# bschrag620/PyRad

Measured on NVIDIA B200. Metric: line-gridpoint evals/s, higher is better.
Workload: dtype f32

## Files before the change

pyrad_b200/csrc/common.cuh:

```cuda
#pragma once
#include <cuda_runtime.h>
#include <stdint.h>
#include <math.h>

namespace prb {

constexpr double kBoltz = 1.38064852E-23;
constexpr double cLight = 299792458.0;
constexpr double hPlanck = 6.62607004e-34;
constexpr double kPi = 3.141592653589793;
constexpr double kT0 = 296.0;
constexpr double kP0 = 1013.25;
constexpr double kAvogadro = 6.022140857E23;

constexpr int REGIME_GAUSS = 0, REGIME_LORENTZ = 1, REGIME_VOIGT = 2;

struct GroupParams {
    double conc;
    double dopp;
    double qratio;
    double weight;
};

struct DevState {
    unsigned int reserved0;
    unsigned int flags;
    unsigned int tile_counter;
    unsigned int pad;
};

constexpr unsigned int FLAG_OVERFLOW = 1u, FLAG_NONFINITE = 2u;

#ifndef PRB_K2_CONSUMERS
#define PRB_K2_CONSUMERS 8
#endif
#ifndef PRB_K2_ACC_SMEM
#define PRB_K2_ACC_SMEM 0
#endif
constexpr int K2_CONSUMERS = PRB_K2_CONSUMERS;
constexpr int K2_THREADS = 32 * (K2_CONSUMERS + 1);
#ifndef PRB_K2_CHUNK
#define PRB_K2_CHUNK 768
#endif
#ifndef PRB_K2_STAGES
#define PRB_K2_STAGES 3
#endif
#ifndef PRB_K2_MIN_CTAS
#define PRB_K2_MIN_CTAS 2
#endif
constexpr int K2_CHUNK = PRB_K2_CHUNK;
constexpr int K2_STAGES = PRB_K2_STAGES;
constexpr int K2_MIN_CTAS = PRB_K2_MIN_CTAS;
constexpr int K2_FLUSH = 64;
constexpr float K2_SENTINEL = 3.0e38f;

__device__ __forceinline__ uint32_t smem_u32(const void *p) {
    return (uint32_t)__cvta_generic_to_shared(p);
}
__device__ __forceinline__ void mbar_init(uint64_t *bar, uint32_t count) {
    asm volatile("mbarrier.init.shared::cta.b64 [%0], %1;" ::"r"(smem_u32(bar)), "r"(count) : "memory");
}
__device__ __forceinline__ void mbar_expect_tx(uint64_t *bar, uint32_t bytes) {
    asm volatile("mbarrier.arrive.expect_tx.shared::cta.b64 _, [%0], %1;" ::"r"(smem_u32(bar)), "r"(bytes)
                 : "memory");
}
__device__ __forceinline__ void mbar_arrive(uint64_t *bar) {
    asm volatile("mbarrier.arrive.shared::cta.b64 _, [%0];" ::"r"(smem_u32(bar)) : "memory");
}
__device__ __forceinline__ void mbar_wait(uint64_t *bar, uint32_t parity) {
    asm volatile(
        "{\n"
        ".reg .pred p;\n"
        "WAIT_%=:\n"
        "mbarrier.try_wait.parity.shared::cta.b64 p, [%0], %1;\n"
        "@p bra DONE_%=;\n"
        "bra WAIT_%=;\n"
        "DONE_%=:\n"
        "}\n" ::"r"(smem_u32(bar)),
        "r"(parity)
        : "memory");
}
__device__ __forceinline__ void mbar_wait_parked(uint64_t *bar, uint32_t parity) {
    asm volatile(
        "{\n"
        ".reg .pred p;\n"
        "WAITP_%=:\n"
        "mbarrier.try_wait.parity.shared::cta.b64 p, [%0], %1, %2;\n"
        "@p bra DONEP_%=;\n"
        "bra WAITP_%=;\n"
        "DONEP_%=:\n"
        "}\n" ::"r"(smem_u32(bar)),
        "r"(parity), "r"(4000u)
        : "memory");
}
__device__ __forceinline__ void tma_bulk_g2s(void *dst, const void *src, uint32_t bytes, uint64_t *bar) {
    asm volatile(
        "cp.async.bulk.shared::cluster.global.mbarrier::complete_tx::bytes [%0], [%1], %2, [%3];" ::"r"(
            smem_u32(dst)),
        "l"(src), "r"(bytes), "r"(smem_u32(bar))
        : "memory");
}

}
```

pyrad_b200/csrc/k2_line_sum.cuh:

```cuda
#pragma once
#include "common.cuh"
#include "k3_stream.cuh"

namespace prb {

__device__ __forceinline__ float rcp_approx(float x) {
    float r;
    asm("rcp.approx.ftz.f32 %0, %1;" : "=f"(r) : "f"(x));
    return r;
}
__device__ __forceinline__ float ex2_approx(float x) {
    float r;
    asm("ex2.approx.ftz.f32 %0, %1;" : "=f"(r) : "f"(x));
    return r;
}

__device__ __forceinline__ void tma_bulk_s2g(void *dst, const void *src, uint32_t bytes) {
    asm volatile("cp.async.bulk.global.shared::cta.bulk_group [%0], [%1], %2;" ::"l"(dst), "r"(smem_u32(src)), "r"(bytes)
                 : "memory");
}
__device__ __forceinline__ void consumer_barrier() {
    asm volatile("bar.sync 1, %0;" ::"n"(K2_CONSUMERS * 32) : "memory");
}

__device__ __forceinline__ int warp_lower_bound(const int32_t *__restrict__ idx, int lo, int hi, long long key) {
    const int lane = threadIdx.x & 31;
    while (hi > lo) {
        const int span = hi - lo;
        const int step = (span + 31) >> 5;
        int pos = lo + (lane + 1) * step - 1;
        pos = pos < hi - 1 ? pos : hi - 1;
        const bool less = (long long)__ldg(idx + pos) < key;
        const unsigned m = __ballot_sync(0xffffffffu, less);
        const int c = __popc(m);
        int nlo = lo, nhi = hi;
        if (c > 0) { int p = lo + c * step - 1; p = p < hi - 1 ? p : hi - 1; nlo = p + 1; }
        if (c < 32) { int p = lo + (c + 1) * step - 1; p = p < hi - 1 ? p : hi - 1; nhi = p; }
        lo = nlo;
        hi = nhi;
    }
    return lo;
}

constexpr int K2_MAX_XSC = 8;
struct K2Layer {
    const float4 *recA;
    const float4 *recB;
    const float *recD;
    void *out;
    double inv_scale;
    int l_begin, l_end;
    int wm;
    int pad;
    double xsc_w[K2_MAX_XSC];
};

constexpr int K2_MAX_PEERS = 8;
constexpr int K2_MAX_DST = K2_MAX_PEERS + 1;
struct K2Fuse {
    int enabled;
    int n_dst;
    float neg_depth_log2e;
    float c2_over_t, c2_over_tsurf;
    long long n_total;
    double x0, dx, x_last;
    float *rad[K2_MAX_DST];
    float *trans[K2_MAX_DST];
};

struct K2Args {
    const K2Layer *layers;
    int n_layers;
    const int32_t *idx;
    long long i_begin;
    int n_chunk;
    int n_tiles;
    int tile_base;
    const int2 *tile_bounds;
    int variant;
    int out_mode;
    DevState *st;
    K2Fuse fuse;
    const double *far_lag;
    float far_delta[16];
    const double *far_lag2;
    float far_delta2[16];
    const double *xsc_sigma;
    long long xsc_ld;
    int n_xsc;
    int parts;
    double *part_sums;
    unsigned int *part_count;
};

__device__ __forceinline__ double k2_add_xsc(const K2Args &a, const K2Layer *L, int i, double v) {
    for (int t = 0; t < a.n_xsc; ++t)
        v = __dadd_rn(v, __dmul_rn(__ldg(a.xsc_sigma + (long long)t * a.xsc_ld + i), __ldg(&L->xsc_w[t])));
    return v;
}

constexpr int K2_FAR_NODES = 16;
constexpr int K2_FAR_RADIUS_SPANS = 1;
constexpr int K2_FAR_SUBGROUPS = 64 / K2_FAR_NODES;
constexpr int K2_FAR_FLUSH = 16;
#ifndef PRB_K2_FAR2_SPANS
#define PRB_K2_FAR2_SPANS 8
#endif
constexpr int K2_FAR2_SPANS = PRB_K2_FAR2_SPANS;
#ifndef PRB_K2_FAR2_ENABLE
#define PRB_K2_FAR2_ENABLE 1
#endif
constexpr bool K2_FAR2 = PRB_K2_FAR2_ENABLE != 0;
constexpr int K2_FAR2_MIN_DOMAINS = 4;
static_assert(K2_CONSUMERS % K2_FAR2_SPANS == 0, "a tile is a whole number of level-2 domains");

struct K2Desc {
    int tile0;
    int cnt;
    int flags;
    int layer;
    int part;
};
constexpr int K2_FIRST = 1, K2_LAST = 2, K2_END = 4;

struct K2Smem {
    float4 rA[K2_STAGES][K2_CHUNK];
    float4 rB[K2_STAGES][K2_CHUNK];
    float rD[K2_STAGES][K2_CHUNK];
    K2Desc desc[K2_STAGES];
    uint64_t full[K2_STAGES];
    uint64_t empty[K2_STAGES];
    double far2[2][K2_CONSUMERS][K2_FAR_NODES];
    double2 faracc[2][K2_CONSUMERS * 32];
    int part_last;
};

template <int P>
__host__ __device__ constexpr size_t K2_SMEM_BASE() {
    return ((sizeof(K2Smem) + (PRB_K2_ACC_SMEM ? sizeof(double) * P * K2_CONSUMERS * 32 : 0)) + 127) & ~size_t(127);
}
template <int P>
__host__ __device__ constexpr size_t K2_SMEM_BYTES(bool peer_staging) {
    return K2_SMEM_BASE<P>() + (peer_staging ? sizeof(float) * 2 * K2_CONSUMERS * 32 * P : 0);
}

template <int H>
struct Acc {
    float2 fi[H];
    float2 a32[H];
#if PRB_K2_ACC_SMEM
    double *a64;
    __device__ __forceinline__ double &acc(int p) { return a64[p * (K2_CONSUMERS * 32)]; }
#else
    double a64[2 * H];
    __device__ __forceinline__ double &acc(int p) { return a64[p]; }
#endif
    __device__ __forceinline__ void flush() {
#pragma unroll
        for (int j = 0; j < H; ++j) {
            acc(2 * j) += (double)a32[j].x;
            acc(2 * j + 1) += (double)a32[j].y;
            a32[j] = make_float2(0.f, 0.f);
        }
    }
};

__device__ __forceinline__ float2 splat(float v) { return make_float2(v, v); }
__device__ __forceinline__ float2 lo2(const float4 &v) { return make_float2(v.x, v.y); }
__device__ __forceinline__ float2 hi2(const float4 &v) { return make_float2(v.z, v.w); }

template <int H, bool MASKED>
__device__ __forceinline__ void triple_step(const float4 &a1, const float4 &a2, const float4 &a3, const float2 &B1,
                                            const float2 &B2, const float2 &B3, float wmf, Acc<H> &s) {
    const float2 nf1 = lo2(a1), nf2 = lo2(a2), nf3 = lo2(a3);
#pragma unroll
    for (int h = 0; h < H; ++h) {
        const float2 e1 = __fadd2_rn(s.fi[h], nf1);
        const float2 e2 = __fadd2_rn(s.fi[h], nf2);
        const float2 e3 = __fadd2_rn(s.fi[h], nf3);
        const float2 q1 = __ffma2_rn(e1, e1, B1);
        const float2 q2 = __ffma2_rn(e2, e2, B2);
        const float2 q3 = __ffma2_rn(e3, e3, B3);
        float2 A1 = hi2(a1), A2 = hi2(a2), A3 = hi2(a3);
        if (MASKED) {
            A1.x = fabsf(e1.x) <= wmf ? A1.x : 0.f;
            A1.y = fabsf(e1.y) <= wmf ? A1.y : 0.f;
            A2.x = fabsf(e2.x) <= wmf ? A2.x : 0.f;
            A2.y = fabsf(e2.y) <= wmf ? A2.y : 0.f;
            A3.x = fabsf(e3.x) <= wmf ? A3.x : 0.f;
            A3.y = fabsf(e3.y) <= wmf ? A3.y : 0.f;
        }
        const float2 p23 = __fmul2_rn(q2, q3);
        const float2 t = __ffma2_rn(A3, q2, __fmul2_rn(A2, q3));
        const float2 num = __ffma2_rn(q1, t, __fmul2_rn(A1, p23));
        const float2 den = __fmul2_rn(q1, p23);
        const float2 r = make_float2(rcp_approx(den.x), rcp_approx(den.y));
        s.a32[h] = __ffma2_rn(num, r, s.a32[h]);
    }
}

__device__ __forceinline__ float2 ldB(const float4 *sB, int j) { return *reinterpret_cast<const float2 *>(sB + j); }

template <int H, bool MASKED>
__device__ __forceinline__ void lorentz_paired(const float4 *sA, const float4 *sB, int js, int je, float wmf,
                                               Acc<H> &s) {
    const int n = je - js;
    if (n <= 0) return;
    int j = js;
    const int n6 = (n / 6) * 6;
    const int jq = js + n6;
    if (n6) {
        float4 xa1 = sA[j], xa2 = sA[j + 1], xa3 = sA[j + 2], ya1 = sA[j + 3], ya2 = sA[j + 4], ya3 = sA[j + 5];
        float2 xb1 = ldB(sB, j), xb2 = ldB(sB, j + 1), xb3 = ldB(sB, j + 2);
        float2 yb1 = ldB(sB, j + 3), yb2 = ldB(sB, j + 4), yb3 = ldB(sB, j + 5);
        int since = 0;
        for (j += 6; j < jq; j += 6) {
            triple_step<H, MASKED>(xa1, xa2, xa3, xb1, xb2, xb3, wmf, s);
            xa1 = sA[j]; xa2 = sA[j + 1]; xa3 = sA[j + 2];
            xb1 = ldB(sB, j); xb2 = ldB(sB, j + 1); xb3 = ldB(sB, j + 2);
            triple_step<H, MASKED>(ya1, ya2, ya3, yb1, yb2, yb3, wmf, s);
            ya1 = sA[j + 3]; ya2 = sA[j + 4]; ya3 = sA[j + 5];
            yb1 = ldB(sB, j + 3); yb2 = ldB(sB, j + 4); yb3 = ldB(sB, j + 5);
            if (++since == K2_FLUSH / 6) { s.flush(); since = 0; }
        }
        triple_step<H, MASKED>(xa1, xa2, xa3, xb1, xb2, xb3, wmf, s);
        triple_step<H, MASKED>(ya1, ya2, ya3, yb1, yb2, yb3, wmf, s);
    }
    for (j = jq; j < je; j += 3) {
        const float4 a1 = sA[j];
        const float2 B1 = ldB(sB, j);
        const float4 z = make_float4(a1.x, a1.y, 0.f, 0.f);
        const bool h2 = j + 1 < je, h3 = j + 2 < je;
        triple_step<H, MASKED>(a1, h2 ? sA[j + 1] : z, h3 ? sA[j + 2] : z, B1, h2 ? ldB(sB, j + 1) : B1,
                               h3 ? ldB(sB, j + 2) : B1, wmf, s);
    }
    s.flush();
}

#ifndef PRB_K2_GAUSS_PAIR_H
#define PRB_K2_GAUSS_PAIR_H 2
#endif
constexpr int K2_GAUSS_PAIR_H = PRB_K2_GAUSS_PAIR_H;

template <int H, bool MASKED>
__device__ __forceinline__ void gauss_pass(const float4 *sA, const float4 *sB, const float *sD, int js, int je,
                                           float wbf, float we1f, float wmf, Acc<H> &s) {
    int since = 0;
    for (int jb = js; jb < je; jb += 32) {
        const int jt = jb + (int)(threadIdx.x & 31);
        bool hit = false;
        if (jt < je) {
            const float dg = sD[jt];
            const float f = -sA[jt].x;
            hit = (dg >= 0.f) && (f + dg >= wbf) && (f - dg <= we1f);
        }
        unsigned int m = __ballot_sync(0xffffffffu, hit);
        auto one = [&](const float4 &b, float nf1) {
            const float2 nf = splat(nf1), C2 = splat(b.w);
#pragma unroll
            for (int h = 0; h < H; ++h) {
                const float2 e = __fadd2_rn(s.fi[h], nf);
                const float2 arg = __fmul2_rn(C2, __fmul2_rn(e, e));
                float2 g = splat(b.z);
                if (MASKED) {
                    g.x = fabsf(e.x) <= wmf ? b.z : 0.f;
                    g.y = fabsf(e.y) <= wmf ? b.z : 0.f;
                }
                s.a32[h] = __ffma2_rn(g, make_float2(ex2_approx(arg.x), ex2_approx(arg.y)), s.a32[h]);
            }
        };
        while (m) {
            const int j = jb + __ffs(m) - 1;
            m &= m - 1;
            if (H <= K2_GAUSS_PAIR_H && m) {
                const int j2 = jb + __ffs(m) - 1;
                m &= m - 1;
                const float4 b1 = sB[j], b2 = sB[j2];
                const float n1 = sA[j].x, n2 = sA[j2].x;
                const float2 nfa = splat(n1), nfb = splat(n2), Ca = splat(b1.w), Cb = splat(b2.w);
                float2 ta[H], tb[H], ga[H], gb[H];
#pragma unroll
                for (int h = 0; h < H; ++h) {
                    const float2 ea = __fadd2_rn(s.fi[h], nfa), eb = __fadd2_rn(s.fi[h], nfb);
                    const float2 xa = __fmul2_rn(Ca, __fmul2_rn(ea, ea)), xb = __fmul2_rn(Cb, __fmul2_rn(eb, eb));
                    ga[h] = splat(b1.z);
                    gb[h] = splat(b2.z);
                    if (MASKED) {
                        ga[h].x = fabsf(ea.x) <= wmf ? b1.z : 0.f;
                        ga[h].y = fabsf(ea.y) <= wmf ? b1.z : 0.f;
                        gb[h].x = fabsf(eb.x) <= wmf ? b2.z : 0.f;
                        gb[h].y = fabsf(eb.y) <= wmf ? b2.z : 0.f;
                    }
                    ta[h] = make_float2(ex2_approx(xa.x), ex2_approx(xa.y));
                    tb[h] = make_float2(ex2_approx(xb.x), ex2_approx(xb.y));
                }
#pragma unroll
                for (int h = 0; h < H; ++h) s.a32[h] = __ffma2_rn(gb[h], tb[h], __ffma2_rn(ga[h], ta[h], s.a32[h]));
                since += 2;
                if (since >= K2_FLUSH) { s.flush(); since = 0; }
                continue;
            }
            one(sB[j], sA[j].x);
            if (++since >= K2_FLUSH) { s.flush(); since = 0; }
        }
    }
    if (since) s.flush();
}

struct FarAcc {
    double v0, v1;
};
__device__ __forceinline__ float2 far_triple(const float4 &a1, const float4 &a2, const float4 &a3, const float2 &B1,
                                             const float2 &B2, const float2 &B3, const float2 &A1, const float2 &A2,
                                             const float2 &A3, const float2 &wb2, const float2 &del, const float2 &part) {
    const float2 e1 = __fadd2_rn(__fadd2_rn(wb2, lo2(a1)), del);
    const float2 e2 = __fadd2_rn(__fadd2_rn(wb2, lo2(a2)), del);
    const float2 e3 = __fadd2_rn(__fadd2_rn(wb2, lo2(a3)), del);
    const float2 q1 = __ffma2_rn(e1, e1, B1);
    const float2 q2 = __ffma2_rn(e2, e2, B2);
    const float2 q3 = __ffma2_rn(e3, e3, B3);
    const float2 p23 = __fmul2_rn(q2, q3);
    const float2 t = __ffma2_rn(A3, q2, __fmul2_rn(A2, q3));
    const float2 num = __ffma2_rn(q1, t, __fmul2_rn(A1, p23));
    const float2 den = __fmul2_rn(q1, p23);
    const float2 r = make_float2(rcp_approx(den.x), rcp_approx(den.y));
    return __ffma2_rn(num, r, part);
}
template <int G>
__device__ __forceinline__ void far_pass(const float4 *sA, const float4 *sB, int js, int je, float wbf, float2 del,
                                         double2 *acc, int sub) {
    const int n = je - js;
    if (n <= 0) return;
    const double2 acc0 = *acc;
    FarAcc fa{acc0.x, acc0.y};
    const float2 wb2 = splat(wbf);
    const float2 zero = make_float2(0.f, 0.f);
    int full = n / (3 * G);
    const float4 *pa = sA + js + sub;
    const float4 *pb = sB + js + sub;
    while (full > 0) {
        const int m = min(full, K2_FAR_FLUSH);
        float2 part = zero;
#pragma unroll 2
        for (int i = 0; i < m; ++i) {
            const float4 a1 = pa[0], a2 = pa[G], a3 = pa[2 * G];
            const float2 B1 = ldB(pb, 0), B2 = ldB(pb, G), B3 = ldB(pb, 2 * G);
            part = far_triple(a1, a2, a3, B1, B2, B3, hi2(a1), hi2(a2), hi2(a3), wb2, del, part);
            pa += 3 * G;
            pb += 3 * G;
        }
        fa.v0 += (double)part.x;
        fa.v1 += (double)part.y;
        full -= m;
    }
    const int j0 = js + (n / (3 * G)) * (3 * G);
    if (j0 < je) {
        const int j1 = j0 + sub, j2 = j1 + G, j3 = j1 + 2 * G;
        const int k1 = min(j1, je - 1), k2 = min(j2, je - 1), k3 = min(j3, je - 1);
        const float4 a1 = sA[k1], a2 = sA[k2], a3 = sA[k3];
        const float2 A1 = j1 < je ? hi2(a1) : zero, A2 = j2 < je ? hi2(a2) : zero, A3 = j3 < je ? hi2(a3) : zero;
        const float2 part = far_triple(a1, a2, a3, ldB(sB, k1), ldB(sB, k2), ldB(sB, k3), A1, A2, A3, wb2, del, zero);
        fa.v0 += (double)part.x;
        fa.v1 += (double)part.y;
    }
    *acc = make_double2(fa.v0, fa.v1);
}

template <int H>
__device__ __forceinline__ void general_all(const float4 *sA, const float4 *sB, int cnt, float wmf, Acc<H> &s) {
    for (int jb = 0; jb < cnt; jb += K2_FLUSH) {
        const int jend = min(jb + K2_FLUSH, cnt);
        for (int j = jb; j < jend; ++j) {
            const float4 a = sA[j], b = sB[j];
#pragma unroll
            for (int h = 0; h < H; ++h) {
                const float ex = s.fi[h].x + a.x, ey = s.fi[h].y + a.x;
                const float e2x = ex * ex, e2y = ey * ey;
                float tx = a.z * rcp_approx(e2x + b.x), ty = a.z * rcp_approx(e2y + b.x);
                tx = fmaf(b.z, ex2_approx(b.w * e2x), tx);
                ty = fmaf(b.z, ex2_approx(b.w * e2y), ty);
                s.a32[h].x += (fabsf(ex) <= wmf) ? tx : 0.f;
                s.a32[h].y += (fabsf(ey) <= wmf) ? ty : 0.f;
            }
        }
        s.flush();
    }
}

template <int P, bool FAR, bool SPLIT>
__device__ __forceinline__ void k2_line_sum_body(const K2Args &a) {
    static_assert(P >= 2 && P % 2 == 0, "points per thread must be even (packed FP32x2)");
    static_assert(!FAR || P == 4 || P == 8, "far-field tables exist for 128- and 256-point spans");
    constexpr int H = P / 2;
    constexpr int TILE = K2_CONSUMERS * 32 * P;
    constexpr int SPAN = 32 * P;
    extern __shared__ __align__(128) unsigned char smem_raw[];
    K2Smem &sm = *reinterpret_cast<K2Smem *>(smem_raw);
    const int tid = threadIdx.x, lane = tid & 31, warp = tid >> 5;

    if (tid == 0) {
        for (int s = 0; s < K2_STAGES; ++s) {
            mbar_init(&sm.full[s], 1);
            mbar_init(&sm.empty[s], K2_CONSUMERS);
        }
        asm volatile("fence.mbarrier_init.release.cluster;" ::: "memory");
        asm volatile("fence.proxy.async.shared::cta;" ::: "memory");
    }
    __syncthreads();

    if (warp == K2_CONSUMERS) {
        uint32_t it = 0;
        auto slot_acquire = [&](uint32_t &stage) {
            stage = it % K2_STAGES;
            mbar_wait_parked(&sm.empty[stage], ((it / K2_STAGES) & 1) ^ 1);
        };
        const int parts = (SPLIT && a.parts > 1) ? a.parts : 1;
        const int n_items = a.n_layers * a.n_tiles * parts;
        while (true) {
            int item = 0;
            if (lane == 0) item = (int)atomicAdd(&a.st->tile_counter, 1u);
            item = __shfl_sync(0xffffffffu, item, 0);
            if (item >= n_items) break;
            const int n_lt = a.n_layers * a.n_tiles;
            const int pidx = item / n_lt;
            const int lt = item - pidx * n_lt;
            const int half = parts >> 1, step = pidx >> 2, r = pidx & 3;
            const int part = parts < 4 ? pidx : (r == 0 ? half - 1 - step : r == 1 ? half + step : r == 2 ? step : parts - 1 - step);
            const int layer = lt / a.n_tiles;
            const int tile = a.tile_base + lt - layer * a.n_tiles;
            const K2Layer *L = a.layers + layer;
            const int wm = __ldg(&L->wm), l_begin = __ldg(&L->l_begin), l_end = __ldg(&L->l_end);
            const float4 *recA = L->recA;
            const float4 *recB = L->recB;
            const float *recD = L->recD;
            const int tile0 = tile * TILE;
            const long long k_lo = a.i_begin + tile0 - wm;
            const long long k_hi = a.i_begin + tile0 + TILE - 1 + wm + 1;
            int lo = warp_lower_bound(a.idx, l_begin, l_end, k_lo);
            const int hi = warp_lower_bound(a.idx, lo, l_end, k_hi);
            lo &= ~3;
            const int nch = hi > lo ? (hi - lo + K2_CHUNK - 1) / K2_CHUNK : 1;
            const int c0 = (int)((long long)part * nch / parts), c1 = (int)((long long)(part + 1) * nch / parts);
            const int cn = c1 > c0 ? c1 - c0 : 1;
            for (int k = 0; k < cn; ++k, ++it) {
                const int c = c0 + k;
                uint32_t stage;
                slot_acquire(stage);
                if (lane == 0) {
                    const int first = lo + c * K2_CHUNK;
                    const int cnt = c1 > c0 ? max(min(K2_CHUNK, hi - first), 0) : 0;
                    sm.desc[stage] = K2Desc{tile0, cnt, (k == 0 ? K2_FIRST : 0) | (k == cn - 1 ? K2_LAST : 0), layer, part};
                    if (cnt > 0) {
                        const uint32_t ce = (uint32_t)((cnt + 3) & ~3);
                        mbar_expect_tx(&sm.full[stage], ce * 36u);
                        tma_bulk_g2s(sm.rA[stage], recA + first, ce * 16u, &sm.full[stage]);
                        tma_bulk_g2s(sm.rB[stage], recB + first, ce * 16u, &sm.full[stage]);
                        tma_bulk_g2s(sm.rD[stage], recD + first, ce * 4u, &sm.full[stage]);
                    } else {
                        mbar_arrive(&sm.full[stage]);
                    }
                }
                __syncwarp();
            }
        }
        uint32_t stage;
        slot_acquire(stage);
        if (lane == 0) {
            sm.desc[stage] = K2Desc{0, 0, K2_END, 0, 0};
            mbar_arrive(&sm.full[stage]);
        }
        return;
    }

    float wmf = 0.f;
    Acc<H> s;
#pragma unroll
    for (int h = 0; h < H; ++h) { s.a32[h] = make_float2(0.f, 0.f); s.fi[h] = make_float2(0.f, 0.f); }
#if PRB_K2_ACC_SMEM
    s.a64 = reinterpret_cast<double *>(smem_raw + sizeof(K2Smem)) + tid;
#endif
#pragma unroll
    for (int p = 0; p < P; ++p) s.acc(p) = 0.0;
    int wb = 0;
    float wbf = 0.f, we1f = 0.f;
    double2 *far = &sm.faracc[0][tid];
    double2 *far2 = &sm.faracc[1][tid];
    float dbf = 0.f;
    uint32_t tile_par = 0;
    bool use2 = false;

    for (uint32_t it = 0;; ++it) {
        const uint32_t stage = it % K2_STAGES;
        mbar_wait(&sm.full[stage], (it / K2_STAGES) & 1);
        const K2Desc d = sm.desc[stage];
        if (d.flags & K2_END) {
            if (tid == 0) asm volatile("cp.async.bulk.wait_group 0;" ::: "memory");
            break;
        }
        if (d.flags & K2_FIRST) {
            wmf = (float)__ldg(&a.layers[d.layer].wm);
            wb = d.tile0 + warp * SPAN;
            wbf = (float)wb;
            we1f = (float)(wb + SPAN - 1);
#pragma unroll
            for (int h = 0; h < H; ++h) {
                s.a32[h] = make_float2(0.f, 0.f);
                s.fi[h] = make_float2((float)(wb + lane + 64 * h), (float)(wb + lane + 64 * h + 32));
            }
#pragma unroll
            for (int p = 0; p < P; ++p) s.acc(p) = 0.0;
            if (FAR) {
                *far = make_double2(0.0, 0.0);
                *far2 = make_double2(0.0, 0.0);
            }
            dbf = (float)(d.tile0 + (warp / K2_FAR2_SPANS) * (K2_FAR2_SPANS * SPAN));
            use2 = FAR && K2_FAR2 && wmf >= (float)(K2_FAR2_MIN_DOMAINS * K2_FAR2_SPANS * SPAN);
        }
        const int cnt = d.cnt;
        const float4 *sA = sm.rA[stage];
        const float4 *sB = sm.rB[stage];
        const float *sD = sm.rD[stage];

        if (a.variant == 0) {
            general_all<H>(sA, sB, cnt, wmf, s);
        } else if (cnt > 0) {
            float dgl = 0.f;
            for (int j = lane; j < cnt; j += 32) dgl = fmaxf(dgl, sD[j]);
            const float dgmax = __uint_as_float(__reduce_max_sync(0xffffffffu, __float_as_uint(dgl)));
            const float t0 = wbf - wmf;
            const float t5 = we1f + 1.f + wmf;
            float t1 = we1f - wmf, t4 = wbf + wmf + 1.f;
            if (t1 >= t4) { t1 = t5; t4 = t5; }
            const float g0 = fmaxf(wbf - dgmax, t0);
            const float g1 = fminf(we1f + 1.f + dgmax, t5);
            const float tfl = wbf + (float)((SPAN - 1) / 2 - K2_FAR_RADIUS_SPANS * SPAN);
            const float tfr = wbf + (float)(SPAN / 2 + K2_FAR_RADIUS_SPANS * SPAN);
            int b1, b4, bg0, bg1;
            if (FAR) {
                static_assert(K2_CHUNK <= 1024, "one level-1 sample per lane");
                const float f1 = -sA[min(32 * lane + 31, cnt - 1)].x;
                const bool v1 = 32 * lane < cnt;
                auto below = [&](float t) -> int {
                    const int nb = __popc(__ballot_sync(0xffffffffu, v1 && f1 < t));
                    const int j2 = 32 * nb + lane;
                    const bool l2 = j2 < cnt && -sA[min(j2, cnt - 1)].x < t;
                    return min(32 * nb, cnt) + __popc(__ballot_sync(0xffffffffu, l2));
                };
                constexpr int S2 = K2_FAR2_SPANS * SPAN;
                const int kp = lane & (K2_FAR_NODES / 2 - 1);
                const int sub = lane / (K2_FAR_NODES / 2);
                const float2 del = make_float2(a.far_delta[2 * kp], a.far_delta[2 * kp + 1]);
                const float2 del2 = make_float2(a.far_delta2[2 * kp], a.far_delta2[2 * kp + 1]);
                const int sub2 = (warp % K2_FAR2_SPANS) * K2_FAR_SUBGROUPS + sub;
                const float u1 = dbf + (float)(S2 - 1) - wmf, u4 = dbf + wmf + 1.f;
                const bool l2on = use2 && u1 < u4;
                b1 = below(t1);
                lorentz_paired<H, true>(sA, sB, below(t0), b1, wmf, s);
                b4 = below(t4);
                const int bfl = min(max(below(tfl), b1), b4);
                if (l2on) {
                    const int c4 = below(u4);
                    const int c1 = min(below(u1), c4);
                    const int cfl = min(max(below(dbf + (float)((S2 - 1) / 2 - K2_FAR_RADIUS_SPANS * S2)), c1), c4);
                    const int l1a = min(max(c1, b1), bfl), l1b = min(max(cfl, l1a), bfl);
                    far_pass<K2_FAR_SUBGROUPS>(sA, sB, b1, l1a, wbf, del, far, sub);
                    far_pass<K2_FAR2_SPANS * K2_FAR_SUBGROUPS>(sA, sB, c1, cfl, dbf, del2, far2, sub2);
                    far_pass<K2_FAR_SUBGROUPS>(sA, sB, l1b, bfl, wbf, del, far, sub);
                } else {
                    far_pass<K2_FAR_SUBGROUPS>(sA, sB, b1, bfl, wbf, del, far, sub);
                }
                const int bfr = min(max(below(tfr + 1.f), bfl), b4);
                lorentz_paired<H, false>(sA, sB, bfl, bfr, wmf, s);
                if (l2on) {
                    const int c4 = below(u4);
                    const int c1 = min(below(u1), c4);
                    const int cfl = min(max(below(dbf + (float)((S2 - 1) / 2 - K2_FAR_RADIUS_SPANS * S2)), c1), c4);
                    const int cfr = min(max(below(dbf + (float)(S2 / 2 + K2_FAR_RADIUS_SPANS * S2) + 1.f), cfl), c4);
                    const int r1a = min(max(cfr, bfr), b4), r1b = min(max(c4, r1a), b4);
                    far_pass<K2_FAR_SUBGROUPS>(sA, sB, bfr, r1a, wbf, del, far, sub);
                    far_pass<K2_FAR2_SPANS * K2_FAR_SUBGROUPS>(sA, sB, cfr, c4, dbf, del2, far2, sub2);
                    far_pass<K2_FAR_SUBGROUPS>(sA, sB, r1b, b4, wbf, del, far, sub);
                } else {
                    far_pass<K2_FAR_SUBGROUPS>(sA, sB, bfr, b4, wbf, del, far, sub);
                }
                lorentz_paired<H, true>(sA, sB, b4, below(t5), wmf, s);
                bg0 = below(g0);
                bg1 = below(g1);
            } else {
                int c0 = 0, c1 = 0, c4 = 0, c5 = 0, cg0 = 0, cg1 = 0;
                for (int j = lane; j < cnt; j += 32) {
                    const float f = -sA[j].x;
                    c0 += f < t0; c1 += f < t1; c4 += f < t4; c5 += f < t5; cg0 += f < g0; cg1 += f < g1;
                }
                const int b0 = __reduce_add_sync(0xffffffffu, c0);
                b1 = __reduce_add_sync(0xffffffffu, c1);
                b4 = __reduce_add_sync(0xffffffffu, c4);
                const int b5 = __reduce_add_sync(0xffffffffu, c5);
                bg0 = __reduce_add_sync(0xffffffffu, cg0);
                bg1 = __reduce_add_sync(0xffffffffu, cg1);
                lorentz_paired<H, true>(sA, sB, b0, b1, wmf, s);
                lorentz_paired<H, false>(sA, sB, b1, b4, wmf, s);
                lorentz_paired<H, true>(sA, sB, b4, b5, wmf, s);
            }
            if (dgmax > 0.f) {
                gauss_pass<H, true>(sA, sB, sD, bg0, min(bg1, b1), wbf, we1f, wmf, s);
                gauss_pass<H, false>(sA, sB, sD, max(bg0, b1), min(bg1, b4), wbf, we1f, wmf, s);
                gauss_pass<H, true>(sA, sB, sD, max(bg0, b4), bg1, wbf, we1f, wmf, s);
            }
        }
        __syncwarp();
        if (lane == 0) mbar_arrive(&sm.empty[stage]);

        if (d.flags & K2_LAST) {
            const K2Layer *L = a.layers + d.layer;
            const double inv_scale = __ldg(&L->inv_scale);
            void *out = L->out;
            const bool bulk = a.fuse.enabled && a.fuse.n_dst > 1 && d.tile0 + TILE <= a.n_chunk;
            float *stage_rad = reinterpret_cast<float *>(smem_raw + K2_SMEM_BASE<P>());
            float *stage_tr = stage_rad + TILE;
            if (bulk) {
                if (tid == 0) asm volatile("cp.async.bulk.wait_group.read 0;" ::: "memory");
                consumer_barrier();
            }
            if (FAR) {
                double v0 = far->x, v1 = far->y, w0 = far2->x, w1 = far2->y;
#pragma unroll
                for (int o = K2_FAR_NODES / 2; o < 32; o <<= 1) {
                    v0 += __shfl_xor_sync(0xffffffffu, v0, o);
                    v1 += __shfl_xor_sync(0xffffffffu, v1, o);
                    w0 += __shfl_xor_sync(0xffffffffu, w0, o);
                    w1 += __shfl_xor_sync(0xffffffffu, w1, o);
                }
                if (use2 && lane < K2_FAR_NODES / 2) {
                    sm.far2[tile_par][warp][2 * lane] = w0;
                    sm.far2[tile_par][warp][2 * lane + 1] = w1;
                }
                if (use2) consumer_barrier();
                double dn = 0.0;
                if (use2 && lane < K2_FAR_NODES) {
                    const int wd = (warp / K2_FAR2_SPANS) * K2_FAR2_SPANS;
#pragma unroll
                    for (int q = 0; q < K2_FAR2_SPANS; ++q) dn += sm.far2[tile_par][wd + q][lane];
                }
                if (use2) tile_par ^= 1u;
                constexpr int S2 = K2_FAR2_SPANS * SPAN;
                const double *lw2base = a.far_lag2 + (warp % K2_FAR2_SPANS) * SPAN + lane;
#pragma unroll 2
                for (int k = 0; k < K2_FAR_NODES; ++k) {
                    const double fk = __shfl_sync(0xffffffffu, (k & 1) ? v1 : v0, k >> 1);
                    const double *lw = a.far_lag + k * SPAN + lane;
#pragma unroll
                    for (int p = 0; p < P; ++p) s.acc(p) = fma(fk, __ldg(lw + 32 * p), s.acc(p));
                    if (use2) {
                        const double gk = __shfl_sync(0xffffffffu, dn, k);
                        const double *lw2 = lw2base + k * S2;
#pragma unroll
                        for (int p = 0; p < P; ++p) s.acc(p) = fma(gk, __ldg(lw2 + 32 * p), s.acc(p));
                    }
                }
            }
            bool finish = true;
            if (SPLIT && a.parts > 1) {
                const int lt = d.layer * a.n_tiles + (d.tile0 / TILE - a.tile_base);
                double *mine = a.part_sums + ((size_t)lt * a.parts + d.part) * TILE + warp * SPAN + lane;
#pragma unroll
                for (int p = 0; p < P; ++p) __stcg(mine + 32 * p, s.acc(p));
                __threadfence();
                consumer_barrier();
                if (tid == 0) sm.part_last = atomicAdd(a.part_count + lt, 1u) == (unsigned int)(a.parts - 1);
                consumer_barrier();
                finish = sm.part_last != 0;
                if (finish) {
                    __threadfence();
                    const double *all = a.part_sums + (size_t)lt * a.parts * TILE + warp * SPAN + lane;
#pragma unroll
                    for (int p = 0; p < P; ++p) {
                        double v = 0.0;
                        for (int q = 0; q < a.parts; ++q) v += __ldcg(all + (size_t)q * TILE + 32 * p);
                        s.acc(p) = v;
                    }
                }
            }
            if (finish) {
#pragma unroll
                for (int p = 0; p < P; ++p) {
                    const int i = wb + 32 * p + lane;
                    if (i < a.n_chunk) {
                        const double v = k2_add_xsc(a, L, i, s.acc(p) * inv_scale);
                        if (a.out_mode == 0) reinterpret_cast<double *>(out)[i] = v;
                        else reinterpret_cast<float *>(out)[i] = (float)v;
                        if (a.fuse.enabled) {
                            const double x = axis_value(a.i_begin + i, a.fuse.n_total, a.fuse.x0, a.fuse.dx, a.fuse.x_last);
                            const float nu = (float)x;
                            const float a3 = (float)(2E8 * hPlanck * (cLight * cLight) * (x * x * x));
                            const float e = (float)v * a.fuse.neg_depth_log2e;
                            const float b = planck_f32(a3, a.fuse.c2_over_t * nu);
                            const float rad = k3_fold_step(planck_f32(a3, a.fuse.c2_over_tsurf * nu), e, b);
                            const float tr = exp2f(0.f + e);
                            if (bulk) {
                                stage_rad[i - d.tile0] = rad;
                                stage_tr[i - d.tile0] = tr;
                            } else {
#pragma unroll 1
                                for (int dst = 0; dst < a.fuse.n_dst; ++dst) {
                                    a.fuse.rad[dst][i] = rad;
                                    a.fuse.trans[dst][i] = tr;
                                }
                            }
                        }
                    }
                }
                if (bulk) {
                    asm volatile("fence.proxy.async.shared::cta;" ::: "memory");
                    consumer_barrier();
                    if (tid == 0) {
#pragma unroll 1
                        for (int dst = 0; dst < a.fuse.n_dst; ++dst) {
                            tma_bulk_s2g(a.fuse.rad[dst] + d.tile0, stage_rad, TILE * 4u);
                            tma_bulk_s2g(a.fuse.trans[dst] + d.tile0, stage_tr, TILE * 4u);
                        }
                        asm volatile("cp.async.bulk.commit_group;" ::: "memory");
                    }
                }
            }
        }
    }
}

template <int P, bool SPLIT = false>
__global__ void __launch_bounds__(K2_THREADS, K2_MIN_CTAS) k2_line_sum(const K2Args a) {
    k2_line_sum_body<P, false, SPLIT>(a);
}
template <int P, bool SPLIT = false>
__global__ void __launch_bounds__(K2_THREADS, K2_MIN_CTAS) k2_line_sum_far(const K2Args a) {
    k2_line_sum_body<P, true, SPLIT>(a);
}

}
```

Measured before the change: 4990 billion.

## Offload per-slot line bounds and Gaussian hit masks to producer warp

For non-FAR paths with P>=8, the producer warp builds a per-stage index after each chunk lands. It holds binary-searched line bounds for every consumer span plus a bitmask of Gaussian hits, and publishes it through a new 'ready' mbarrier. Consumers read these precomputed bounds and masks instead of scanning all lines with per-warp counting reductions and ballots. This moves redundant per-warp work onto the otherwise idle producer warp, at the cost of extra shared memory, a serial producer stage that could delay consumers, and more complex barrier interleaving.

Measured after the change: 5053 billion, median of 6. 1.01x the previous value.

```diff
diff --git a/pyrad_b200/csrc/common.cuh b/pyrad_b200/csrc/common.cuh
--- a/pyrad_b200/csrc/common.cuh
+++ b/pyrad_b200/csrc/common.cuh
@@ -93,6 +93,19 @@
         "r"(parity), "r"(4000u)
         : "memory");
 }
+__device__ __forceinline__ bool mbar_test(uint64_t *bar, uint32_t parity) {
+    uint32_t done;
+    asm volatile(
+        "{\n"
+        ".reg .pred p;\n"
+        "mbarrier.test_wait.parity.shared::cta.b64 p, [%1], %2;\n"
+        "selp.u32 %0, 1, 0, p;\n"
+        "}\n"
+        : "=r"(done)
+        : "r"(smem_u32(bar)), "r"(parity)
+        : "memory");
+    return done != 0;
+}
 __device__ __forceinline__ void tma_bulk_g2s(void *dst, const void *src, uint32_t bytes, uint64_t *bar) {
     asm volatile(
         "cp.async.bulk.shared::cluster.global.mbarrier::complete_tx::bytes [%0], [%1], %2, [%3];" ::"r"(
diff --git a/pyrad_b200/csrc/k2_line_sum.cuh b/pyrad_b200/csrc/k2_line_sum.cuh
--- a/pyrad_b200/csrc/k2_line_sum.cuh
+++ b/pyrad_b200/csrc/k2_line_sum.cuh
@@ -123,6 +123,12 @@
 };
 constexpr int K2_FIRST = 1, K2_LAST = 2, K2_END = 4;
 
+struct K2SlotIndex {
+    int b0, b1, b4, b5, bg0, bg1;
+};
+static_assert(K2_CHUNK % 32 == 0, "Gaussian hit masks: whole 32-line words per slot");
+constexpr int K2_GMASK_WORDS = K2_CHUNK / 32;
+
 struct K2Smem {
     float4 rA[K2_STAGES][K2_CHUNK];
     float4 rB[K2_STAGES][K2_CHUNK];
@@ -130,6 +136,9 @@
     K2Desc desc[K2_STAGES];
     uint64_t full[K2_STAGES];
     uint64_t empty[K2_STAGES];
+    uint64_t ready[K2_STAGES];
+    K2SlotIndex index[K2_STAGES][K2_CONSUMERS];
+    uint32_t gmask[K2_STAGES][K2_CONSUMERS][K2_GMASK_WORDS];
     double far2[2][K2_CONSUMERS][K2_FAR_NODES];
     double2 faracc[2][K2_CONSUMERS * 32];
     int part_last;
@@ -242,19 +251,26 @@
 #endif
 constexpr int K2_GAUSS_PAIR_H = PRB_K2_GAUSS_PAIR_H;
 
-template <int H, bool MASKED>
-__device__ __forceinline__ void gauss_pass(const float4 *sA, const float4 *sB, const float *sD, int js, int je,
-                                           float wbf, float we1f, float wmf, Acc<H> &s) {
+__device__ __forceinline__ bool gauss_hit(float f, float dg, float wbf, float we1f) {
+    return (dg >= 0.f) && (f + dg >= wbf) && (f - dg <= we1f);
+}
+
+template <int H, bool MASKED, bool INDEXED>
+__device__ __forceinline__ void gauss_pass(const float4 *sA, const float4 *sB, const float *sD, const uint32_t *gm,
+                                           int js, int je, float wbf, float we1f, float wmf, Acc<H> &s) {
     int since = 0;
     for (int jb = js; jb < je; jb += 32) {
-        const int jt = jb + (int)(threadIdx.x & 31);
-        bool hit = false;
-        if (jt < je) {
-            const float dg = sD[jt];
-            const float f = -sA[jt].x;
-            hit = (dg >= 0.f) && (f + dg >= wbf) && (f - dg <= we1f);
-        }
-        unsigned int m = __ballot_sync(0xffffffffu, hit);
+        unsigned int m;
+        if (INDEXED) {
+            const int k = jb >> 5;
+            m = __funnelshift_r(gm[k], gm[min(k + 1, K2_GMASK_WORDS - 1)], jb & 31);
+            if (je - jb < 32) m &= (1u << (je - jb)) - 1u;
+        } else {
+            const int jt = jb + (int)(threadIdx.x & 31);
+            bool hit = false;
+            if (jt < je) hit = gauss_hit(-sA[jt].x, sD[jt], wbf, we1f);
+            m = __ballot_sync(0xffffffffu, hit);
+        }
         auto one = [&](const float4 &b, float nf1) {
             const float2 nf = splat(nf1), C2 = splat(b.w);
 #pragma unroll
@@ -387,6 +403,71 @@
     }
 }
 
+__device__ __forceinline__ float slot_dgmax(const float *sD, int cnt) {
+    float dgl = 0.f;
+    for (int j = (int)(threadIdx.x & 31); j < cnt; j += 32) dgl = fmaxf(dgl, sD[j]);
+    return __uint_as_float(__reduce_max_sync(0xffffffffu, __float_as_uint(dgl)));
+}
+
+struct K2Thresholds {
+    float t0, t1, t4, t5, g0, g1;
+};
+__device__ __forceinline__ K2Thresholds span_thresholds(float wbf, float we1f, float wmf, float dgmax) {
+    const float t0 = wbf - wmf;
+    const float t5 = we1f + 1.f + wmf;
+    float t1 = we1f - wmf, t4 = wbf + wmf + 1.f;
+    if (t1 >= t4) { t1 = t5; t4 = t5; }
+    const float g0 = fmaxf(wbf - dgmax, t0);
+    const float g1 = fminf(we1f + 1.f + dgmax, t5);
+    return K2Thresholds{t0, t1, t4, t5, g0, g1};
+}
+
+__device__ __forceinline__ int slot_below(const float4 *sA, int cnt, float f1, bool v1, float t) {
+    const int lane = threadIdx.x & 31;
+    const int nb = __popc(__ballot_sync(0xffffffffu, v1 && f1 < t));
+    const int j2 = 32 * nb + lane;
+    const bool l2 = j2 < cnt && -sA[min(j2, cnt - 1)].x < t;
+    return min(32 * nb, cnt) + __popc(__ballot_sync(0xffffffffu, l2));
+}
+
+template <int SPAN>
+__device__ __forceinline__ void k2_slot_index(K2Smem &sm, int stage, int tile0, float wmf) {
+    constexpr int NB = sizeof(K2SlotIndex) / sizeof(int);
+    const int lane = threadIdx.x & 31;
+    const float4 *sA = sm.rA[stage];
+    const float *sD = sm.rD[stage];
+    const int cnt = sm.desc[stage].cnt;
+    const float dgmax = slot_dgmax(sD, cnt);
+    int *bounds = reinterpret_cast<int *>(sm.index[stage]);
+    for (int q = lane; q < NB * K2_CONSUMERS; q += 32) {
+        const int w = q / NB, c = q - w * NB;
+        const int wb = tile0 + w * SPAN;
+        const K2Thresholds t = span_thresholds((float)wb, (float)(wb + SPAN - 1), wmf, dgmax);
+        const float th = c == 0 ? t.t0 : c == 1 ? t.t1 : c == 2 ? t.t4 : c == 3 ? t.t5 : (c == 4 || dgmax <= 0.f) ? t.g0 : t.g1;
+        int lo = 0, hi = cnt;
+        while (lo < hi) {
+            const int mid = (lo + hi) >> 1;
+            if (-sA[mid].x < th) lo = mid + 1;
+            else hi = mid;
+        }
+        bounds[q] = lo;
+    }
+    __syncwarp();
+    if (dgmax > 0.f) {
+#pragma unroll 1
+        for (int w = 0; w < K2_CONSUMERS; ++w) {
+            const int bg0 = sm.index[stage][w].bg0, bg1 = sm.index[stage][w].bg1;
+            const int wb = tile0 + w * SPAN;
+            for (int k = bg0 >> 5; 32 * k < bg1; ++k) {
+                const int j = 32 * k + lane;
+                const bool hit = j < cnt && gauss_hit(-sA[min(j, cnt - 1)].x, sD[min(j, cnt - 1)], (float)wb, (float)(wb + SPAN - 1));
+                const uint32_t m = __ballot_sync(0xffffffffu, hit);
+                if (lane == 0) sm.gmask[stage][w][k] = m;
+            }
+        }
+    }
+}
+
 template <int P, bool FAR, bool SPLIT>
 __device__ __forceinline__ void k2_line_sum_body(const K2Args &a) {
     static_assert(P >= 2 && P % 2 == 0, "points per thread must be even (packed FP32x2)");
@@ -394,6 +475,7 @@
     constexpr int H = P / 2;
     constexpr int TILE = K2_CONSUMERS * 32 * P;
     constexpr int SPAN = 32 * P;
+    constexpr bool INDEX = !FAR && P >= 8;
     extern __shared__ __align__(128) unsigned char smem_raw[];
     K2Smem &sm = *reinterpret_cast<K2Smem *>(smem_raw);
     const int tid = threadIdx.x, lane = tid & 31, warp = tid >> 5;
@@ -402,6 +484,7 @@
         for (int s = 0; s < K2_STAGES; ++s) {
             mbar_init(&sm.full[s], 1);
             mbar_init(&sm.empty[s], K2_CONSUMERS);
+            if (INDEX) mbar_init(&sm.ready[s], 1);
         }
         asm volatile("fence.mbarrier_init.release.cluster;" ::: "memory");
         asm volatile("fence.proxy.async.shared::cta;" ::: "memory");
@@ -410,13 +493,35 @@
 
     if (warp == K2_CONSUMERS) {
         uint32_t it = 0;
+        uint32_t ix = 0;
+        auto index_next = [&]() {
+            const uint32_t stage = ix % K2_STAGES;
+            mbar_wait_parked(&sm.full[stage], (ix / K2_STAGES) & 1);
+            const K2Desc d = sm.desc[stage];
+            if (d.cnt > 0) k2_slot_index<SPAN>(sm, stage, d.tile0, (float)__ldg(&a.layers[d.layer].wm));
+            __syncwarp();
+            if (lane == 0) mbar_arrive(&sm.ready[stage]);
+            ++ix;
+        };
+        auto landed = [&]() {
+            return __shfl_sync(0xffffffffu, (int)mbar_test(&sm.full[ix % K2_STAGES], (ix / K2_STAGES) & 1), 0) != 0;
+        };
+        auto index_landed = [&]() {
+            if (INDEX)
+                while (ix < it && landed()) index_next();
+        };
         auto slot_acquire = [&](uint32_t &stage) {
             stage = it % K2_STAGES;
-            mbar_wait_parked(&sm.empty[stage], ((it / K2_STAGES) & 1) ^ 1);
+            const uint32_t par = ((it / K2_STAGES) & 1) ^ 1;
+            if (INDEX)
+                while (ix < it && (landed() || !__shfl_sync(0xffffffffu, (int)mbar_test(&sm.empty[stage], par), 0)))
+                    index_next();
+            mbar_wait_parked(&sm.empty[stage], par);
         };
         const int parts = (SPLIT && a.parts > 1) ? a.parts : 1;
         const int n_items = a.n_layers * a.n_tiles * parts;
         while (true) {
+            index_landed();
             int item = 0;
             if (lane == 0) item = (int)atomicAdd(&a.st->tile_counter, 1u);
             item = __shfl_sync(0xffffffffu, item, 0);
@@ -469,6 +574,9 @@
             sm.desc[stage] = K2Desc{0, 0, K2_END, 0, 0};
             mbar_arrive(&sm.full[stage]);
         }
+        __syncwarp();
+        if (INDEX)
+            for (++it; ix < it;) index_next();
         return;
     }
 
@@ -491,7 +599,7 @@
 
     for (uint32_t it = 0;; ++it) {
         const uint32_t stage = it % K2_STAGES;
-        mbar_wait(&sm.full[stage], (it / K2_STAGES) & 1);
+        mbar_wait(INDEX ? &sm.ready[stage] : &sm.full[stage], (it / K2_STAGES) & 1);
         const K2Desc d = sm.desc[stage];
         if (d.flags & K2_END) {
             if (tid == 0) asm volatile("cp.async.bulk.wait_group 0;" ::: "memory");
@@ -524,28 +632,14 @@
         if (a.variant == 0) {
             general_all<H>(sA, sB, cnt, wmf, s);
         } else if (cnt > 0) {
-            float dgl = 0.f;
-            for (int j = lane; j < cnt; j += 32) dgl = fmaxf(dgl, sD[j]);
-            const float dgmax = __uint_as_float(__reduce_max_sync(0xffffffffu, __float_as_uint(dgl)));
-            const float t0 = wbf - wmf;
-            const float t5 = we1f + 1.f + wmf;
-            float t1 = we1f - wmf, t4 = wbf + wmf + 1.f;
-            if (t1 >= t4) { t1 = t5; t4 = t5; }
-            const float g0 = fmaxf(wbf - dgmax, t0);
-            const float g1 = fminf(we1f + 1.f + dgmax, t5);
-            const float tfl = wbf + (float)((SPAN - 1) / 2 - K2_FAR_RADIUS_SPANS * SPAN);
-            const float tfr = wbf + (float)(SPAN / 2 + K2_FAR_RADIUS_SPANS * SPAN);
-            int b1, b4, bg0, bg1;
             if (FAR) {
-                static_assert(K2_CHUNK <= 1024, "one level-1 sample per lane");
+                const float dgmax = slot_dgmax(sD, cnt);
+                const K2Thresholds th = span_thresholds(wbf, we1f, wmf, dgmax);
+                const float tfl = wbf + (float)((SPAN - 1) / 2 - K2_FAR_RADIUS_SPANS * SPAN);
+                const float tfr = wbf + (float)(SPAN / 2 + K2_FAR_RADIUS_SPANS * SPAN);
                 const float f1 = -sA[min(32 * lane + 31, cnt - 1)].x;
                 const bool v1 = 32 * lane < cnt;
-                auto below = [&](float t) -> int {
-                    const int nb = __popc(__ballot_sync(0xffffffffu, v1 && f1 < t));
-                    const int j2 = 32 * nb + lane;
-                    const bool l2 = j2 < cnt && -sA[min(j2, cnt - 1)].x < t;
-                    return min(32 * nb, cnt) + __popc(__ballot_sync(0xffffffffu, l2));
-                };
+                auto below = [&](float t) -> int { return slot_below(sA, cnt, f1, v1, t); };
                 constexpr int S2 = K2_FAR2_SPANS * SPAN;
                 const int kp = lane & (K2_FAR_NODES / 2 - 1);
                 const int sub = lane / (K2_FAR_NODES / 2);
@@ -554,9 +648,9 @@
                 const int sub2 = (warp % K2_FAR2_SPANS) * K2_FAR_SUBGROUPS + sub;
                 const float u1 = dbf + (float)(S2 - 1) - wmf, u4 = dbf + wmf + 1.f;
                 const bool l2on = use2 && u1 < u4;
-                b1 = below(t1);
-                lorentz_paired<H, true>(sA, sB, below(t0), b1, wmf, s);
-                b4 = below(t4);
+                const int b1 = below(th.t1);
+                lorentz_paired<H, true>(sA, sB, below(th.t0), b1, wmf, s);
+                const int b4 = below(th.t4);
                 const int bfl = min(max(below(tfl), b1), b4);
                 if (l2on) {
                     const int c4 = below(u4);
@@ -583,29 +677,49 @@
                 } else {
                     far_pass<K2_FAR_SUBGROUPS>(sA, sB, bfr, b4, wbf, del, far, sub);
                 }
-                lorentz_paired<H, true>(sA, sB, b4, below(t5), wmf, s);
-                bg0 = below(g0);
-                bg1 = below(g1);
+                lorentz_paired<H, true>(sA, sB, b4, below(th.t5), wmf, s);
+                if (dgmax > 0.f) {
+                    const int bg0 = below(th.g0), bg1 = below(th.g1);
+                    gauss_pass<H, true, false>(sA, sB, sD, nullptr, bg0, min(bg1, b1), wbf, we1f, wmf, s);
+                    gauss_pass<H, false, false>(sA, sB, sD, nullptr, max(bg0, b1), min(bg1, b4), wbf, we1f, wmf, s);
+                    gauss_pass<H, true, false>(sA, sB, sD, nullptr, max(bg0, b4), bg1, wbf, we1f, wmf, s);
+                }
+            } else if (INDEX) {
+                const K2SlotIndex &x = sm.index[stage][warp];
+                auto uni = [](int v) { return (int)__reduce_max_sync(0xffffffffu, (unsigned)v); };
+                const int b1 = uni(x.b1), b4 = uni(x.b4);
+                const uint32_t *gm = sm.gmask[stage][warp];
+                lorentz_paired<H, true>(sA, sB, uni(x.b0), b1, wmf, s);
+                lorentz_paired<H, false>(sA, sB, b1, b4, wmf, s);
+                lorentz_paired<H, true>(sA, sB, b4, uni(x.b5), wmf, s);
+                const int bg0 = uni(x.bg0), bg1 = uni(x.bg1);
+                if (bg0 < bg1) {
+                    gauss_pass<H, true, true>(sA, sB, sD, gm, bg0, min(bg1, b1), wbf, we1f, wmf, s);
+                    gauss_pass<H, false, true>(sA, sB, sD, gm, max(bg0, b1), min(bg1, b4), wbf, we1f, wmf, s);
+                    gauss_pass<H, true, true>(sA, sB, sD, gm, max(bg0, b4), bg1, wbf, we1f, wmf, s);
+                }
             } else {
+                const float dgmax = slot_dgmax(sD, cnt);
+                const K2Thresholds th = span_thresholds(wbf, we1f, wmf, dgmax);
                 int c0 = 0, c1 = 0, c4 = 0, c5 = 0, cg0 = 0, cg1 = 0;
                 for (int j = lane; j < cnt; j += 32) {
                     const float f = -sA[j].x;
-                    c0 += f < t0; c1 += f < t1; c4 += f < t4; c5 += f < t5; cg0 += f < g0; cg1 += f < g1;
+                    c0 += f < th.t0; c1 += f < th.t1; c4 += f < th.t4; c5 += f < th.t5; cg0 += f < th.g0; cg1 += f < th.g1;
                 }
                 const int b0 = __reduce_add_sync(0xffffffffu, c0);
-                b1 = __reduce_add_sync(0xffffffffu, c1);
-                b4 = __reduce_add_sync(0xffffffffu, c4);
+                const int b1 = __reduce_add_sync(0xffffffffu, c1);
+                const int b4 = __reduce_add_sync(0xffffffffu, c4);
                 const int b5 = __reduce_add_sync(0xffffffffu, c5);
-                bg0 = __reduce_add_sync(0xffffffffu, cg0);
-                bg1 = __reduce_add_sync(0xffffffffu, cg1);
+                const int bg0 = __reduce_add_sync(0xffffffffu, cg0);
+                const int bg1 = __reduce_add_sync(0xffffffffu, cg1);
                 lorentz_paired<H, true>(sA, sB, b0, b1, wmf, s);
                 lorentz_paired<H, false>(sA, sB, b1, b4, wmf, s);
                 lorentz_paired<H, true>(sA, sB, b4, b5, wmf, s);
-            }
-            if (dgmax > 0.f) {
-                gauss_pass<H, true>(sA, sB, sD, bg0, min(bg1, b1), wbf, we1f, wmf, s);
-                gauss_pass<H, false>(sA, sB, sD, max(bg0, b1), min(bg1, b4), wbf, we1f, wmf, s);
-                gauss_pass<H, true>(sA, sB, sD, max(bg0, b4), bg1, wbf, we1f, wmf, s);
+                if (dgmax > 0.f) {
+                    gauss_pass<H, true, false>(sA, sB, sD, nullptr, bg0, min(bg1, b1), wbf, we1f, wmf, s);
+                    gauss_pass<H, false, false>(sA, sB, sD, nullptr, max(bg0, b1), min(bg1, b4), wbf, we1f, wmf, s);
+                    gauss_pass<H, true, false>(sA, sB, sD, nullptr, max(bg0, b4), bg1, wbf, we1f, wmf, s);
+                }
             }
         }
         __syncwarp();
```
